# Weobe/plonky2-ecdsa

Hardware: AMD Instinct MI355X
Metric: secp256k1 ECDSA witness fills/sec at batch=2^16, 1/2/4/8 MI355X; bit-exact (higher is better)
Workload: dtype u64

## Files before the change

__graft_entry__.py:

```python
import os
import subprocess
import sys

ROOT = os.path.dirname(os.path.abspath(__file__))
sys.path.insert(0, ROOT)


def build() -> None:
    import plonky2_ecdsa_amd as p2e
    p2e.build(verbose=True)
    subprocess.check_call(["make", "-s", "-C", os.path.join(ROOT, "oracle"), "libp2e_oracle.so"])
    subprocess.check_call(["make", "-s", "-C", os.path.join(ROOT, "tests", "emu")])
    subprocess.check_call(["make", "-s", "-C", os.path.join(ROOT, "tests", "probe")])
    subprocess.check_call(["make", "-s", "-C", os.path.join(ROOT, "tests", "probe_hash")])
    p2e.lib()
    assert p2e.schedule_num_cols(p2e.PROGRAM_VERIFY) == p2e.VERIFY_COLS


def smoke() -> None:
    import numpy as np
    import torch
    import plonky2_ecdsa_amd as p2e
    sys.path.insert(0, os.path.join(ROOT, "oracle"))
    import oracle_c

    n = 64
    sigs = p2e.synth_signatures(seed=1, n=n)
    ctx = p2e.Context(device=0, phase_timing=True)
    dev = [torch.from_numpy(a).cuda() for a in sigs]
    cols, err, valid, bad = ctx.ecdsa_verify_witness_batch(*dev)
    torch.cuda.synchronize()
    assert bad == 0 and bool(valid.cpu().numpy().all()), "synthetic signatures must verify"
    ref_cols, ref_aux, ref_err, ref_flags = oracle_c.verify_witness_aux(*sigs)
    got = cols.cpu().numpy().view(np.uint64)
    assert np.array_equal(got, ref_cols), "GPU witness differs from the oracle"
    phases = ctx.last_phase_ms()
    aux, aerr, abad = ctx.aux_witness_batch(p2e.PROGRAM_VERIFY, dev[4], cols, n=n, ld=cols.stride(0))
    torch.cuda.synchronize()
    assert abad == 0 and np.array_equal(aux.cpu().numpy().view(np.uint64), ref_aux), "aux columns differ from the oracle"
    print(f"smoke ok: {n} fills x ({p2e.VERIFY_COLS} + {p2e.VERIFY_AUX_COLS}) columns bit-exact vs oracle; phases {phases}")


if __name__ == "__main__":
    build()
    if "--smoke" in sys.argv:
        smoke()
```

plonky2-ecdsa_amd/csrc/p2e_hip.hip:

```cpp
#include <hip/hip_runtime.h>

#include <algorithm>
#include <cstdio>
#include <cstdlib>
#include <cstring>
#include <memory>
#include <mutex>
#include <string>
#include <type_traits>
#include <vector>

#include "../../include/p2e.h"
#include "aux.hpp"
#include "consts.hpp"
#include "device_array.hpp"
#include "knobs.hpp"
#include "launch_plan.hpp"
#include "pipeline.hpp"
#include "prims.hpp"
#include "quad.hpp"
#include "schedule.hpp"
#include "curve_program.hpp"
#include "sign.hpp"
#include "recover.hpp"
#include "pmsm.hpp"
#include "hash.hpp"
#include "wire.hpp"

using namespace p2e;
using host::COMPACT_WIDE;

#ifndef P2E_PART
#define P2E_PART (-1)
#endif
#define P2E_HAS(p) (P2E_PART < 0 || P2E_PART == (p))

constexpr int BS = 256;

template <bool WIDE>
__device__ __forceinline__ size_t lane_sig(size_t first) {
    unsigned t = threadIdx.x;
    size_t base = first + (size_t)blockIdx.x * BS;
    if (WIDE) return base + (t & ~63u) + 2u * (t & 31u) + ((t >> 5) & 1u);
    return base + t;
}
template <int MODE> struct EmitOf;
template <> struct EmitOf<0> { typedef Emit type; };
template <> struct EmitOf<1> { typedef PairEmit type; };
template <> struct EmitOf<2> { typedef CompactEmit type; };
template <> struct EmitOf<3> { typedef CompactPairEmit type; };
template <> struct EmitOf<4> { typedef NullEmit type; };
#if P2E_HAS(1)
template <int MODE>
__global__ __launch_bounds__(BS) void k_scalar(Program G, Buffers B, size_t first) {
    size_t i = lane_sig<(MODE & 1) != 0>(first);
    if ((MODE & 1) || i < B.n) body_scalar<typename EmitOf<MODE>::type>(G, B, i);
}
__global__ __launch_bounds__(BS) void k_chains(Program G, Buffers B, int lo, int hi, int table_affine, int continue_prefix) {
    __builtin_amdgcn_s_setprio(3);
    size_t i = (size_t)blockIdx.x * BS + threadIdx.x;
#ifdef P2E_LDS_FBTAB
    constexpr int MAXW = 36;
    __shared__ Aff s_fb[MAXW * 16];
    const OpDesc first = load_op(B.ops, lo);
    const bool fb = first.kind != OP_DBL && ref_kind(first.ref2) == R_FBTAB && hi - lo <= MAXW;
    const u32 w0 = ref_id(first.ref2);
    if (fb) {
        const int nwin = (hi - lo) < (int)(FB_WINDOWS - w0) ? (hi - lo) : (int)(FB_WINDOWS - w0);
        const u32* src = reinterpret_cast<const u32*>(B.fbtab + (size_t)w0 * 16);
        u32* dst = reinterpret_cast<u32*>(s_fb);
        for (int k = threadIdx.x; k < nwin * 16 * 16; k += BS) dst[k] = src[k];
    }
    __syncthreads();
    if (i < B.n) body_chain_range(G, B, i, lo, hi, table_affine != 0, continue_prefix != 0, fb ? s_fb : nullptr, w0);
#else
    if (i < B.n) body_chain_range(G, B, i, lo, hi, table_affine != 0, continue_prefix != 0);
#endif
}
__global__ __launch_bounds__(BS) void k_chains_quad(Program G, Buffers B, int lo, int hi, int table_affine, int continue_prefix) {
    __builtin_amdgcn_s_setprio(3);
    const size_t g = (size_t)blockIdx.x * BS + threadIdx.x;
    const size_t i = g >> 2;
    if (i < B.n) body_chain_range_quad(G, B, i, (int)(g & 3), lo, hi, table_affine != 0, continue_prefix != 0);
}
__global__ __launch_bounds__(BS) void k_batch_inv_split(Program G, Buffers B, int lo, int hi, int have_prefix, int split_log2) {
    const size_t g = (size_t)blockIdx.x * BS + threadIdx.x;
    const size_t i = g >> split_log2;
    if (i < B.n) body_batch_inv_split(G, B, i, lo, hi, have_prefix != 0, (int)(g & ((1u << split_log2) - 1)), 1 << split_log2);
}
__global__ __launch_bounds__(BS) void k_chain_rows(Program G, Buffers B, int lo, int count) {
    __builtin_amdgcn_s_setprio(3);
    size_t i = (size_t)blockIdx.x * BS + threadIdx.x;
    if (i < B.n) body_chain_rows(G, B, i, lo, (int)gridDim.y, (int)blockIdx.y, count);
}
__global__ __launch_bounds__(BS) void k_batch_inv(Program G, Buffers B, int lo, int hi, int have_prefix) {
    size_t i = (size_t)blockIdx.x * BS + threadIdx.x;
    if (i < B.n) body_batch_inv(G, B, i, lo, hi, have_prefix != 0);
}
template <int MODE>
__global__ __launch_bounds__(BS) void k_expand(Program G, Buffers B, int lo, size_t first) {
#ifdef P2E_EXPAND_PRIO
    __builtin_amdgcn_s_setprio(P2E_EXPAND_PRIO);
#endif
    size_t i = lane_sig<(MODE & 1) != 0>(first);
#ifdef P2E_LDS_FBTAB
    __shared__ Aff s_fb[16];
    const OpDesc op0 = load_op(B.ops, lo + (int)blockIdx.y);
    const bool fb = op0.kind != OP_DBL && ref_kind(op0.ref2) == R_FBTAB;
    if (fb) reinterpret_cast<u32*>(s_fb)[threadIdx.x] = reinterpret_cast<const u32*>(B.fbtab + (size_t)ref_id(op0.ref2) * 16)[threadIdx.x];
    __syncthreads();
    if ((MODE & 1) || i < B.n) body_expand<typename EmitOf<MODE>::type>(G, B, i, lo + (int)blockIdx.y, fb ? s_fb : nullptr);
#else
    if ((MODE & 1) || i < B.n) body_expand<typename EmitOf<MODE>::type>(G, B, i, lo + (int)blockIdx.y);
#endif
}
template <int MODE>
__global__ __launch_bounds__(BS) void k_expand_runs(Program G, Buffers B, int it_first, int run_iters, int it_end, size_t first) {
#ifdef P2E_EXPAND_PRIO
    __builtin_amdgcn_s_setprio(P2E_EXPAND_PRIO);
#endif
    size_t i = lane_sig<(MODE & 1) != 0>(first);
    int it0 = it_first + (int)blockIdx.y * run_iters;
    int it1 = it0 + run_iters < it_end ? it0 + run_iters : it_end;
    if ((MODE & 1) || i < B.n) body_expand_run<typename EmitOf<MODE>::type>(G, B, i, it0, it1);
}
template <int MODE>
__global__ __launch_bounds__(BS) void k_expand_fb_run(Program G, Buffers B, int t_after, size_t first) {
    size_t i = lane_sig<(MODE & 1) != 0>(first);
    if ((MODE & 1) || i < B.n) body_expand_fb_run<typename EmitOf<MODE>::type>(G, B, i, t_after);
}
__global__ __launch_bounds__(BS) void k_verify_check(Program G, Buffers B) {
    size_t i = (size_t)blockIdx.x * BS + threadIdx.x;
    if (i < B.n) body_verify_check(G, B, i);
}
#endif
template <int MODE> struct AuxEmitOf;
template <> struct AuxEmitOf<0> { typedef Emit type; };
template <> struct AuxEmitOf<1> { typedef PairEmit type; };
template <> struct AuxEmitOf<2> { typedef Emit32 type; };
template <> struct AuxEmitOf<3> { typedef PairEmit32 type; };
#if P2E_HAS(0)
template <int MODE>
__global__ __launch_bounds__(BS) void k_aux(AuxArgs A, size_t first) {
    size_t i = lane_sig<(MODE & 1) != 0>(first);
    if ((MODE & 1) || i < A.n) body_aux<typename AuxEmitOf<MODE>::type>(A, (int)blockIdx.y, i);
}
template <int MODE>
__global__ __launch_bounds__(BS) void k_gate(GateArgs A, size_t first) {
    size_t i = lane_sig<(MODE & 1) != 0>(first);
    if ((MODE & 1) || i < A.n) body_gate<typename AuxEmitOf<MODE>::type>(A, (int)blockIdx.y, i);
}
template <int MODE>
__global__ __launch_bounds__(BS) void k_ux(UxArgs A, size_t first) {
    size_t i = lane_sig<(MODE & 1) != 0>(first);
    if ((MODE & 1) || i < A.n) body_ux<typename AuxEmitOf<MODE>::type>(A, (int)blockIdx.y, i);
}
template <int MODE>
__global__ __launch_bounds__(BS) void k_gate_compact(GateArgs A, size_t first) {
    size_t i = lane_sig<(MODE & 1) != 0>(first);
    if ((MODE & 1) || i < A.n) body_gate<typename AuxEmitOf<MODE>::type, true>(A, (int)blockIdx.y, i);
}
template <int MODE>
__global__ __launch_bounds__(BS) void k_ux_compact(UxArgs A, size_t first) {
    size_t i = lane_sig<(MODE & 1) != 0>(first);
    if ((MODE & 1) || i < A.n) body_ux<typename AuxEmitOf<MODE>::type, true>(A, (int)blockIdx.y, i);
}
#endif
static __global__ __launch_bounds__(BS) void k_finalize(const u32* err32, const uint8_t* valid8, uint8_t* err_out,
                                                 uint8_t* valid_out, size_t n, unsigned long long* counter) {
    size_t i = (size_t)blockIdx.x * BS + threadIdx.x;
    bool bad = false;
    if (i < n) {
        u32 e = err32[i];
        bad = e != 0;
        if (err_out) err_out[i] = (uint8_t)e;
        if (valid_out) valid_out[i] = bad ? 0 : valid8[i];
    }
    unsigned long long m = __ballot(bad);
// ... 2510 lines not shown
```

plonky2-ecdsa_amd/csrc/pipeline.hpp:

```cpp
#pragma once
#include "ec29.hpp"
#include "wit.hpp"

namespace p2e {

enum OpKind : uint8_t { OP_ADD = 0, OP_DBL = 1, OP_CADD = 2 };
enum RefKind : uint32_t { R_SLOT = 0, R_CONST = 1, R_DYN = 2, R_FBTAB = 3, R_MSMTAB = 4, R_SELSLOT = 5 };
enum OpFlags : uint8_t { F_Z1ONE = 1, F_Z2ONE = 2, F_CHECK_R = 4, F_NO_AFFINE = 8 };
P2E_HD constexpr u32 make_ref(u32 kind, u32 id) { return (kind << 24) | id; }
P2E_HD constexpr u32 ref_kind(u32 r) { return r >> 24; }
P2E_HD constexpr u32 ref_id(u32 r) { return r & 0xFFFFFFu; }
constexpr uint16_t DYN_CONST_BIT = 0x8000;
constexpr uint16_t SRC_FB_BIT = 0x4000, SRC_SEL_BIT = 0x2000, SRC_ID_MASK = 0x1FFF;

struct OpDesc {
    uint8_t kind;
    uint8_t flags;
    uint16_t cadd_idx;
    u32 ref1, ref2;
    u32 col;
};
static_assert(sizeof(OpDesc) == 16, "load_op reads a descriptor as one 16-byte word");
P2E_HD OpDesc load_op(const OpDesc* ops, int t) {
#if defined(__HIP_DEVICE_COMPILE__)
// ... 219 lines not shown
    return B.fbtab[window * 16 + digit];
}

struct ChainState {
    Jac out, p1;
    uint16_t out_id, p1_id;
    U256 acc;
};
P2E_HD Jac jac_select3(bool c1, const Jac& a, bool c2, const Jac& b, const Jac& c) {
    Jac r;
    r.X = u256_select(c1, a.X, u256_select(c2, b.X, c.X));
    r.Y = u256_select(c1, a.Y, u256_select(c2, b.Y, c.Y));
    r.Z = u256_select(c1, a.Z, u256_select(c2, b.Z, c.Z));
    return r;
}
template <class CV = Secp256k1, bool GENERIC = false>
P2E_HD void body_chain_op(const Program& G, const Buffers& B, size_t i, int t, bool table_affine, ChainState& st,
                          const Aff* lds_fb = nullptr, u32 lds_w0 = 0) {
    typedef typename CV::Fp F;
    const OpDesc op = load_op(B.ops, t);
    size_t o = (size_t)t * B.n + i;
    JacW res;
    uint16_t src1 = resolve_src(G, B, i, op.ref1);
    const bool from_out = src1 == st.out_id, from_p1 = src1 == st.p1_id;
    Jac p1 = st.out;
    if (!(from_out || from_p1)) p1 = load_jac_src(B, i, src1, (op.flags & F_Z1ONE) != 0);
    p1 = jac_select3(from_out, st.out, from_p1, st.p1, p1);
    B.src[(size_t)(2 * t) * B.n + i] = src1;
    if (op.kind == OP_DBL) {
        res = jac_dbl_cv<CV>(p1);
    } else {
        Jac p2;
        u32 digit = 1;
        uint16_t src2;
        bool z2one = (op.flags & F_Z2ONE) != 0;
        if (GENERIC && ref_kind(op.ref2) == R_SELSLOT) {
            digit = B.dig2[(size_t)(ref_id(op.ref2) >> 12) * B.n + i];
            src2 = (uint16_t)(ref_id(op.ref2) & 0xFFFu);
            p2 = load_jac_src(B, i, src2, z2one);
        } else if (ref_kind(op.ref2) == R_FBTAB) {
            Aff a = load_fbtab(B, i, ref_id(op.ref2), digit, lds_fb, lds_w0);
            p2 = jac_from_aff(a);
            src2 = (uint16_t)(SRC_FB_BIT | (ref_id(op.ref2) * 16 + digit));
        } else {
            const bool tab = ref_kind(op.ref2) == R_MSMTAB;
            if (tab) digit = B.dig2[(size_t)ref_id(op.ref2) * B.n + i];
            src2 = resolve_src(G, B, i, op.ref2);
            if (tab && table_affine) {
                p2 = jac_from_aff(load_aff_src(B, i, src2));
                z2one = true;
            } else {
                p2 = load_jac_src(B, i, src2, (op.flags & F_Z2ONE) != 0);
            }
        }
        B.src[(size_t)(2 * t + 1) * B.n + i] = (uint16_t)(src2 | (digit != 0 ? SRC_SEL_BIT : 0));
        if ((op.flags & F_Z1ONE) && z2one)
            res = jac_add_cv<CV, true, true>(p1, p2);
        else if (z2one)
            res = jac_add_cv<CV, false, true>(p1, p2);
        else if (op.flags & F_Z1ONE)
            res = jac_add_cv<CV, true, false>(p1, p2);
        else
            res = jac_add_cv<CV, false, false>(p1, p2);
        if (op.kind == OP_CADD) B.dyn[(size_t)op.cadd_idx * B.n + i] = digit != 0 ? (uint16_t)t : src1;
    }
    if (!(op.flags & F_NO_AFFINE)) {
        B.PX[o] = res.p.X;
        B.PY[o] = res.p.Y;
    }
    B.PZ[o] = res.p.Z;
    B.PW[o] = res.W;
    B.PREF[o] = st.acc;
    U256 z = res.p.Z;
    if (u256_is_zero(z)) {
        err_or(&B.err[i], ERR_INVERSE_OF_ZERO);
        z = u256_small(1);
    }
    st.acc = fe_mul<F>(st.acc, z);
    st.p1 = p1;
    st.p1_id = (op.flags & F_Z1ONE) ? (uint16_t)0xFFFF : src1;
    st.out = res.p;
    st.out_id = (uint16_t)t;
}
struct ChainState29 {
    JacL out, p1;
    uint16_t out_id, p1_id;
    F29 acc;
};
template <bool GENERIC = false>
P2E_HD void body_chain_op29(const Program& G, const Buffers& B, size_t i, int t, bool table_affine, ChainState29& st,
                            const Aff* lds_fb = nullptr, u32 lds_w0 = 0) {
    const OpDesc op = load_op(B.ops, t);
    size_t o = (size_t)t * B.n + i;
    JacWL res;
    uint16_t src1 = resolve_src(G, B, i, op.ref1);
    const bool from_out = src1 == st.out_id, from_p1 = src1 == st.p1_id;
    JacL p1 = st.out;
    if (!(from_out || from_p1)) p1 = jacl_from(load_jac_src(B, i, src1, (op.flags & F_Z1ONE) != 0));
    p1 = jacl_select3(from_out, st.out, from_p1, st.p1, p1);
    B.src[(size_t)(2 * t) * B.n + i] = src1;
    if (op.kind == OP_DBL) {
        res = jac_dbl29(p1);
    } else {
        Jac p2w;
        u32 digit = 1;
        uint16_t src2;
        bool z2one = (op.flags & F_Z2ONE) != 0;
        if (GENERIC && ref_kind(op.ref2) == R_SELSLOT) {
            digit = B.dig2[(size_t)(ref_id(op.ref2) >> 12) * B.n + i];
            src2 = (uint16_t)(ref_id(op.ref2) & 0xFFFu);
            p2w = load_jac_src(B, i, src2, z2one);
        } else if (ref_kind(op.ref2) == R_FBTAB) {
            Aff a = load_fbtab(B, i, ref_id(op.ref2), digit, lds_fb, lds_w0);
            p2w = jac_from_aff(a);
            src2 = (uint16_t)(SRC_FB_BIT | (ref_id(op.ref2) * 16 + digit));
        } else {
            const bool tab = ref_kind(op.ref2) == R_MSMTAB;
            if (tab) digit = B.dig2[(size_t)ref_id(op.ref2) * B.n + i];
            src2 = resolve_src(G, B, i, op.ref2);
            if (tab && table_affine) {
                p2w = jac_from_aff(load_aff_src(B, i, src2));
                z2one = true;
            } else {
                p2w = load_jac_src(B, i, src2, (op.flags & F_Z2ONE) != 0);
            }
        }
        B.src[(size_t)(2 * t + 1) * B.n + i] = (uint16_t)(src2 | (digit != 0 ? SRC_SEL_BIT : 0));
        const JacL p2 = jacl_from(p2w);
        if ((op.flags & F_Z1ONE) && z2one)
            res = jac_add29<true, true>(p1, p2);
        else if (z2one)
            res = jac_add29<false, true>(p1, p2);
        else if (op.flags & F_Z1ONE)
            res = jac_add29<true, false>(p1, p2);
        else
            res = jac_add29<false, false>(p1, p2);
        if (op.kind == OP_CADD) B.dyn[(size_t)op.cadd_idx * B.n + i] = digit != 0 ? (uint16_t)t : src1;
    }
    if (!(op.flags & F_NO_AFFINE)) {
        B.PX[o] = f29_canon_call(res.p.X);
        B.PY[o] = f29_canon_call(res.p.Y);
    }
    const U256 zc = f29_canon_call(res.p.Z);
    B.PZ[o] = zc;
    B.PW[o] = f29_canon_call(res.W);
    B.PREF[o] = f29_canon_call(st.acc);
    const bool z_zero = u256_is_zero(zc);
    if (z_zero) err_or(&B.err[i], ERR_INVERSE_OF_ZERO);
    st.acc = f29_mul_call(st.acc, f29_select(z_zero, f29_small(1), res.p.Z));
    st.p1 = p1;
    st.p1_id = (op.flags & F_Z1ONE) ? (uint16_t)0xFFFF : src1;
    st.out = res.p;
    st.out_id = (uint16_t)t;
}
P2E_HD ChainState29 chain_state29_init(const U256& acc) {
    ChainState29 st;
    st.out_id = st.p1_id = 0xFFFF;
    st.out.X = st.out.Y = st.out.Z = st.p1.X = st.p1.Y = st.p1.Z = f29_small(0);
    st.acc = f29_from_u256(acc);
    return st;
}
template <class CV = Secp256k1>
P2E_HD U256 range_product(const Buffers& B, size_t i, int last) {
    size_t o = (size_t)last * B.n + i;
    U256 z = B.PZ[o];
    if (u256_is_zero(z)) z = u256_small(1);
    return fe_mul<typename CV::Fp>(B.PREF[o], z);
}
template <class CV = Secp256k1, bool GENERIC = false>
P2E_HD void body_chain_range(const Program& G, const Buffers& B, size_t i, int lo, int hi, bool table_affine,
                             bool continue_prefix, const Aff* lds_fb = nullptr, u32 lds_w0 = 0) {
    if (LazyLimbs<CV>::available) {
        ChainState29 st = chain_state29_init(continue_prefix ? range_product<CV>(B, i, lo - 1) : u256_small(1));
        for (int t = lo; t < hi; t++) body_chain_op29<GENERIC>(G, B, i, t, table_affine, st, lds_fb, lds_w0);
        return;
    }
    ChainState st;
    st.out_id = st.p1_id = 0xFFFF;
    st.out.X = st.out.Y = st.out.Z = st.p1.X = st.p1.Y = st.p1.Z = u256_zero();
    st.acc = continue_prefix ? range_product<CV>(B, i, lo - 1) : u256_small(1);
    for (int t = lo; t < hi; t++) body_chain_op<CV, GENERIC>(G, B, i, t, table_affine, st, lds_fb, lds_w0);
}

P2E_HD void body_chain_rows(const Program& G, const Buffers& B, size_t i, int lo, int rows, int row, int count) {
    ChainState29 st = chain_state29_init(u256_small(1));
    for (int j = 0; j < count; j++) body_chain_op29(G, B, i, lo + row + j * rows, false, st);
}

template <class CV = Secp256k1>
P2E_HD void body_verify_check(const Program& G, const Buffers& B, size_t i, int last_op) {
    typedef typename CV::Fp F;
    const size_t o = (size_t)last_op * B.n + i;
    const U256 r = load_packed(B.r, i), X = B.PX[o], Z = B.PZ[o];
    const bool r_lt_p = !geq_mod<F>(r.w);
    if (!(r_lt_p && !u256_is_zero(Z) && u256_eq(fe_mul<F>(r, fe_sqr<F>(Z)), X))) B.valid[i] = 0;
}
P2E_HD void body_verify_check(const Program& G, const Buffers& B, size_t i) {
    body_verify_check<Secp256k1>(G, B, i, G.chain_end[2] - 1);
}

P2E_HD void body_batch_inv29(const Buffers& B, size_t i, int t0, int t1, bool have_prefix, bool uniform_t) {
    U256 accw;
    if (have_prefix) {
        accw = range_product<Secp256k1>(B, i, t1 - 1);
    } else {
        F29 acc = f29_small(1);
        for (int t = t0; t < t1; t++) {
            const size_t o = (size_t)t * B.n + i;
            U256 z = B.PZ[o];
            if (u256_is_zero(z)) z = u256_small(1);
            B.PREF[o] = f29_canon_call(acc);
            acc = f29_mul_call(acc, f29_from_u256(z));
        }
        accw = f29_canon_call(acc);
    }
    F29 inv = f29_from_u256(fe_inv<ModP>(accw));
    struct In {
        U256 z, pref, w, x, y;
        uint8_t flags;
    };
    auto flags_of = [&](int t) { return uniform_t ? load_op(B.ops, t < t0 ? t0 : t).flags : B.ops[t < t0 ? t0 : t].flags; };
    auto fetch = [&](int t, uint8_t fl) {
        In r;
        const size_t o = (size_t)(t < t0 ? t0 : t) * B.n + i;
        const bool aff = !(fl & F_NO_AFFINE);
        r.z = B.PZ[o];
        r.pref = B.PREF[o];
        r.w = B.PW[o];
        r.x = *(aff ? &B.PX[o] : &B.PZ[o]);
        r.y = *(aff ? &B.PY[o] : &B.PZ[o]);
        r.flags = fl;
        return r;
    };
    uint8_t f_nxt = flags_of(t1 - 2);
    In cur = fetch(t1 - 1, flags_of(t1 - 1));
    for (int t = t1 - 1; t >= t0; t--) {
        const uint8_t f_n2 = flags_of(t - 2);
        const In nxt = fetch(t - 1, f_nxt);
        const size_t o = (size_t)t * B.n + i;
        const U256 z = u256_select(u256_is_zero(cur.z), u256_small(1), cur.z);
        const F29 zi = f29_mul_call(inv, f29_from_u256(cur.pref));
        inv = f29_mul_call(inv, f29_from_u256(z));
        B.PW[o] = f29_canon_call(f29_mul_call(f29_from_u256(cur.w), zi));
        if (!(cur.flags & F_NO_AFFINE)) {
            const F29 zi2 = f29_sqr_call(zi);
            const F29 zi3 = f29_mul_call(zi2, zi);
            B.AX[o] = f29_canon_call(f29_mul_call(f29_from_u256(cur.x), zi2));
            B.AY[o] = f29_canon_call(f29_mul_call(f29_from_u256(cur.y), zi3));
        }
        cur = nxt;
        f_nxt = f_n2;
    }
}
template <class CV = Secp256k1>
P2E_HD void body_batch_inv(const Program& G, const Buffers& B, size_t i, int t0, int t1, bool have_prefix, bool uniform_t = true) {
    (void)G;
    typedef typename CV::Fp F;
    if (LazyLimbs<CV>::available) {
        body_batch_inv29(B, i, t0, t1, have_prefix, uniform_t);
        return;
    }
    U256 acc;
    if (have_prefix) {
        acc = range_product<CV>(B, i, t1 - 1);
    } else {
        acc = u256_small(1);
        for (int t = t0; t < t1; t++) {
            size_t o = (size_t)t * B.n + i;
            U256 z = B.PZ[o];
            if (u256_is_zero(z)) z = u256_small(1);
            B.PREF[o] = acc;
            acc = fe_mul<F>(acc, z);
        }
    }
    U256 inv = fe_inv<F>(acc);
    for (int t = t1 - 1; t >= t0; t--) {
        size_t o = (size_t)t * B.n + i;
        U256 z = B.PZ[o];
        if (u256_is_zero(z)) z = u256_small(1);
        U256 zi = fe_mul<F>(inv, B.PREF[o]);
        inv = fe_mul<F>(inv, z);
        B.PW[o] = fe_mul<F>(B.PW[o], zi);
        const uint8_t flags = uniform_t ? load_op(B.ops, t).flags : B.ops[t].flags;
        if (!(flags & F_NO_AFFINE)) {
            U256 zi2 = fe_sqr<F>(zi);
            U256 zi3 = fe_mul<F>(zi2, zi);
            B.AX[o] = fe_mul<F>(B.PX[o], zi2);
            B.AY[o] = fe_mul<F>(B.PY[o], zi3);
        }
    }
}

template <class E, class CV = Secp256k1>
P2E_HD Aff wit_curve_add(E& e, const Aff& p1, const Aff& p2, const U256& vinv, uint8_t& err) {
    U256 u = wit_sub<typename CV::Fp>(e, p2.y, p1.y);
    U256 v = wit_sub<typename CV::Fp>(e, p2.x, p1.x);
    wit_inv_given<typename CV::Fp>(e, v, vinv, err);
    U256 s = wit_mul<typename CV::Fp>(e, u, vinv, err);
    U256 s2 = wit_mul<typename CV::Fp>(e, s, s, err);
    U256 xs = wit_add<typename CV::Fp>(e, p2.x, p1.x);
    Aff r;
    r.x = wit_sub<typename CV::Fp>(e, s2, xs);
    U256 xd = wit_sub<typename CV::Fp>(e, p1.x, r.x);
    U256 pr = wit_mul<typename CV::Fp>(e, s, xd, err);
    r.y = wit_sub<typename CV::Fp>(e, pr, p1.y);
    return r;
}
template <class E, class CV = Secp256k1>
P2E_HD Aff wit_curve_double(E& e, const Aff& p, const U256& vinv, uint8_t& err) {
    U256 dy = wit_add<typename CV::Fp>(e, p.y, p.y);
    wit_inv_given<typename CV::Fp>(e, dy, vinv, err);
    U256 xx = wit_mul<typename CV::Fp>(e, p.x, p.x, err);
    U256 summ[4] = {xx, xx, xx, CV::a()};
    U256 t = wit_add_many<typename CV::Fp, 4>(e, summ);
    U256 l = wit_mul<typename CV::Fp>(e, t, vinv, err);
    U256 l2 = wit_mul<typename CV::Fp>(e, l, l, err);
    U256 xd2 = wit_add<typename CV::Fp>(e, p.x, p.x);
    Aff r;
    r.x = wit_sub<typename CV::Fp>(e, l2, xd2);
    U256 xdf = wit_sub<typename CV::Fp>(e, p.x, r.x);
    U256 lx = wit_mul<typename CV::Fp>(e, l, xdf, err);
    r.y = wit_sub<typename CV::Fp>(e, lx, p.y);
    return r;
}
template <class E, class CV = Secp256k1>
P2E_HD void body_expand(const Program& G, const Buffers& B, size_t i, int t, const Aff* lds_fb = nullptr) {
    const OpDesc op = load_op(B.ops, t);
    uint8_t err = 0;
    E e = E::at(B.sink, i, op.col);
    const uint16_t s1 = B.src[(size_t)(2 * t) * B.n + i];
    const uint16_t s2 = op.kind == OP_DBL ? (uint16_t)0 : B.src[(size_t)(2 * t + 1) * B.n + i];
    U256 vinv = B.PW[(size_t)t * B.n + i];
    Aff p1 = load_aff_src(B, i, s1);
    if (op.kind == OP_DBL) {
// ... 78 lines not shown
```

plonky2-ecdsa_amd/csrc/quad.hpp:

```cpp
#pragma once
#include "pipeline.hpp"
#include "quad29.hpp"

namespace p2e {

#if defined(__HIP_DEVICE_COMPILE__)
template <int J>
__device__ __forceinline__ U256 quad_bcast(const U256& v) {
    U256 r;
    P2E_UNROLL
    for (int k = 0; k < 8; k++)
        r.w[k] = (u32)__builtin_amdgcn_mov_dpp((int)v.w[k], J * 0x55 , 0xF, 0xF, true);
    return r;
}
#endif

template <int USED, bool SQR, class CV = Secp256k1>
P2E_HD void quad_level(int role, const U256& a0, const U256& b0, const U256& a1, const U256& b1, const U256& a2,
                       const U256& b2, const U256& a3, const U256& b3, U256& r0, U256& r1, U256& r2, U256& r3) {
#if defined(__HIP_DEVICE_COMPILE__)
    U256 A = a0, B = b0;
    if (USED > 1) {
        A = u256_select(role == 1, a1, A);
        if (!SQR) B = u256_select(role == 1, b1, B);
// ... 103 lines not shown
P2E_HD QuadRes jac_dbl_quad_cv(int role, const Jac& p, const U256& acc) {
    typedef typename CV::Fp F;
    if (CV::kAZero) return jac_dbl_quad(role, p, acc);
    U256 a, b, yz, zz, c, t0, w, d0, f, y0;
    quad_level<4, false, CV>(role, p.X, p.X, p.Y, p.Y, p.Y, p.Z, p.Z, p.Z, a, b, yz, zz);
    const U256 z3 = fe_add<F>(yz, yz);
    quad_level<3, true, CV>(role, b, b, fe_add<F>(p.X, b), b, zz, b, zz, b, c, t0, w, d0);
    const U256 t = fe_sub<F>(fe_sub<F>(t0, a), c);
    const U256 d = fe_add<F>(t, t);
    const U256 e1 = fe_sub<F>(a, w);
    const U256 e = fe_add<F>(fe_add<F>(e1, e1), e1);
    QuadRes o;
    o.z3_zero = u256_is_zero(z3);
    const U256 zfix = u256_select(o.z3_zero, u256_small(1), z3);
    quad_level<3, false, CV>(role, e, e, acc, zfix, z3, z3, z3, z3, f, o.acc, o.zz3, d0);
    o.res.p.X = fe_sub<F>(f, fe_add<F>(d, d));
    const U256 c2 = fe_add<F>(c, c), c4 = fe_add<F>(c2, c2), c8 = fe_add<F>(c4, c4);
    quad_level<1, false, CV>(role, e, fe_sub<F>(d, o.res.p.X), e, e, e, e, e, e, y0, d0, d0, d0);
    o.res.p.Y = fe_sub<F>(y0, c8);
    o.res.p.Z = z3;
    o.res.W = w;
    o.zz1 = zz;
    return o;
}
template <class CV, bool Z1ONE, bool Z2ONE>
P2E_HD QuadRes jac_add_quad_cv(int role, const Jac& p1, bool have_zz1, const U256& zz1_in, const Jac& p2, const U256& acc) {
    typedef typename CV::Fp F;
    if (CV::kAZero) return jac_add_quad<Z1ONE, Z2ONE>(role, p1, have_zz1, zz1_in, p2, acc);
    U256 zz1 = zz1_in, zz2, z12, z1c, z2c, u1 = p1.X, u2 = p2.X, s1 = p1.Y, s2 = p2.Y, d0, d1;
    if (!Z1ONE && !Z2ONE) {
        quad_level<3, false, CV>(role, p1.Z, p1.Z, p2.Z, p2.Z, p1.Z, p2.Z, p1.Z, p1.Z, zz1, zz2, z12, d0);
    } else if (!Z1ONE) {
        if (!have_zz1) quad_level<1, true, CV>(role, p1.Z, p1.Z, p1.Z, p1.Z, p1.Z, p1.Z, p1.Z, p1.Z, zz1, d0, d1, d0);
    } else if (!Z2ONE) {
        quad_level<1, true, CV>(role, p2.Z, p2.Z, p2.Z, p2.Z, p2.Z, p2.Z, p2.Z, p2.Z, zz2, d0, d1, d0);
    }
    if (!Z1ONE && !Z2ONE) {
        quad_level<4, false, CV>(role, zz1, p1.Z, zz2, p2.Z, p1.X, zz2, p2.X, zz1, z1c, z2c, u1, u2);
    } else if (!Z1ONE) {
        quad_level<2, false, CV>(role, zz1, p1.Z, p2.X, zz1, zz1, zz1, zz1, zz1, z1c, u2, d0, d1);
    } else if (!Z2ONE) {
        quad_level<2, false, CV>(role, zz2, p2.Z, p1.X, zz2, zz2, zz2, zz2, zz2, z2c, u1, d0, d1);
    }
    const U256 h = fe_sub<F>(u2, u1);
    U256 h2, z3;
    if (!Z1ONE && !Z2ONE) {
        quad_level<4, false, CV>(role, p1.Y, z2c, p2.Y, z1c, h, h, z12, h, s1, s2, h2, z3);
    } else if (!Z1ONE) {
        quad_level<3, false, CV>(role, p2.Y, z1c, h, h, p1.Z, h, h, h, s2, h2, z3, d0);
    } else if (!Z2ONE) {
        quad_level<3, false, CV>(role, p1.Y, z2c, h, h, p2.Z, h, h, h, s1, h2, z3, d0);
    } else {
        quad_level<1, true, CV>(role, h, h, h, h, h, h, h, h, h2, d0, d1, d0);
        z3 = h;
    }
    const U256 r = fe_sub<F>(s2, s1);
    U256 h3, v, r2;
    QuadRes o;
    if (!Z1ONE && !Z2ONE) {
        quad_level<4, false, CV>(role, h2, h, u1, h2, r, r, z1c, z2c, h3, v, r2, o.res.W);
    } else {
        quad_level<3, false, CV>(role, h2, h, u1, h2, r, r, r, r, h3, v, r2, d0);
        o.res.W = Z1ONE ? (Z2ONE ? u256_small(1) : z2c) : z1c;
    }
    o.res.p.X = fe_sub<F>(fe_sub<F>(r2, h3), fe_add<F>(v, v));
    o.z3_zero = u256_is_zero(z3);
    const U256 zfix = u256_select(o.z3_zero, u256_small(1), z3);
    U256 t1, t2;
    quad_level<4, false, CV>(role, r, fe_sub<F>(v, o.res.p.X), s1, h3, acc, zfix, z3, z3, t1, t2, o.acc, o.zz3);
    o.res.p.Y = fe_sub<F>(t1, t2);
    o.res.p.Z = z3;
    o.zz1 = zz1;
    return o;
}

struct ChainStateQ {
    Jac out, p1;
    U256 out_zz, p1_zz;
    uint16_t out_id, p1_id;
    uint16_t dyn_idx, dyn_val;
    U256 acc;
};

P2E_HD void settle(U256& v) {
#if defined(__HIP_DEVICE_COMPILE__)
    asm volatile("" : "+v"(v.w[0]), "+v"(v.w[1]), "+v"(v.w[2]), "+v"(v.w[3]), "+v"(v.w[4]), "+v"(v.w[5]), "+v"(v.w[6]), "+v"(v.w[7]));
#else
    (void)v;
#endif
}
P2E_HD void settle(u32& v) {
#if defined(__HIP_DEVICE_COMPILE__)
    asm volatile("" : "+v"(v));
#else
    (void)v;
#endif
}

P2E_HD void quad_store_op(const Buffers& B, size_t i, int role, int t, uint8_t flags, const QuadRes& q, const U256& acc_before) {
    const size_t o = (size_t)t * B.n + i;
    const int r = (flags & F_NO_AFFINE) ? (role | 2) : role;
    uintptr_t bx = (uintptr_t)B.PX, by = (uintptr_t)B.PY, bz = (uintptr_t)B.PZ, bw = (uintptr_t)B.PW;
#if defined(__HIP_DEVICE_COMPILE__)
    asm volatile("" : "+s"(bx), "+s"(by), "+s"(bz), "+s"(bw));
#endif
    U256* const dst = (U256*)(r == 0 ? bx : r == 1 ? by : r == 2 ? bz : bw);
    const U256 val = u256_select(r == 0, q.res.p.X, u256_select(r == 1, q.res.p.Y, u256_select(r == 2, q.res.p.Z, q.res.W)));
    dst[o] = val;
    B.PREF[o] = acc_before;
    if (q.z3_zero) err_or(&B.err[i], ERR_INVERSE_OF_ZERO);
}

P2E_HD void quad_store_op29(const Buffers& B, size_t i, int role, int t, uint8_t flags, const QuadRes29& q) {
    const size_t o = (size_t)t * B.n + i;
    const bool no_affine = (flags & F_NO_AFFINE) != 0;
    uintptr_t bx = (uintptr_t)B.PX, bp = (uintptr_t)B.PREF, bz = (uintptr_t)B.PZ, bw = (uintptr_t)B.PW;
#if defined(__HIP_DEVICE_COMPILE__)
    asm volatile("" : "+s"(bx), "+s"(bp), "+s"(bz), "+s"(bw));
#endif
    U256* const dst = (U256*)(role == 1 ? bp : role == 3 ? bw : (role == 0 && !no_affine) ? bx : bz);
    dst[o] = q.mine;
    if (!no_affine) B.PY[o] = f29_canon(q.p.Y);
    if (q.z3_zero) err_or(&B.err[i], ERR_INVERSE_OF_ZERO);
}

struct P1Sel {
    uint16_t src1;
    Jac p1;
    bool have_zz1;
    U256 zz1;
};
P2E_HD P1Sel quad_first_operand(const Program& G, const Buffers& B, size_t i, const OpDesc& op, const ChainStateQ& st) {
    P1Sel r;
    u32 src1;
    if (ref_kind(op.ref1) == R_DYN && ref_id(op.ref1) == st.dyn_idx) {
        src1 = st.dyn_val;
    } else {
        src1 = resolve_src(G, B, i, op.ref1);
        settle(src1);
    }
    r.src1 = (uint16_t)src1;
    const bool from_out = r.src1 == st.out_id, from_p1 = r.src1 == st.p1_id;
    Jac p1 = st.out;
    if (!(from_out || from_p1)) {
        p1 = load_jac_src(B, i, r.src1, (op.flags & F_Z1ONE) != 0);
        settle(p1.X);
        settle(p1.Y);
        settle(p1.Z);
    }
    r.p1 = jac_select3(from_out, st.out, from_p1, st.p1, p1);
    r.have_zz1 = from_out || from_p1;
    r.zz1 = u256_select(from_out, st.out_zz, st.p1_zz);
    return r;
}

P2E_HD void body_chain_op_quad(const Program& G, const Buffers& B, size_t i, int role, int t, const OpDesc& op, bool table_affine,
                               const P1Sel& s1, ChainStateQ& st) {
    const uint16_t src1 = s1.src1;
    const Jac& p1 = s1.p1;
    if (role == 0) B.src[(size_t)(2 * t) * B.n + i] = src1;
    QuadRes q;
    if (op.kind == OP_DBL) {
        q = jac_dbl_quad(role, p1, st.acc);
    } else {
        Jac p2;
        u32 digit = 1;
        uint16_t src2;
        bool z2one = (op.flags & F_Z2ONE) != 0;
        {
            if (ref_kind(op.ref2) == R_FBTAB) {
                Aff a = load_fbtab(B, i, ref_id(op.ref2), digit);
                p2 = jac_from_aff(a);
                src2 = (uint16_t)(SRC_FB_BIT | (ref_id(op.ref2) * 16 + digit));
            } else {
                const bool tab = ref_kind(op.ref2) == R_MSMTAB;
                if (tab) digit = B.dig2[(size_t)ref_id(op.ref2) * B.n + i];
                src2 = resolve_src(G, B, i, op.ref2);
                if (tab && table_affine) {
                    p2 = jac_from_aff(load_aff_src(B, i, src2));
                    z2one = true;
// ... 298 lines not shown
```

Measured before the change: 6.054 million.

## Add specialized per-lane chain paths for MSM iterations and fixed-base windows

Adds lane-specialized chain kernels for MSM loop iterations (double, double, conditional add) and fixed-base window runs. Both prefetch the next digit and source one iteration ahead and keep the running point in registers instead of resolving and reloading operands per op. Store code is moved into a shared helper, stores are reordered after the arithmetic, and the batch-inverse back pass drops its one-ahead prefetch. Also raises the wave priority of k_batch_inv. This adds code size and register pressure, and the change in load scheduling may not pay off.

```diff
diff --git a/__graft_entry__.py b/__graft_entry__.py
--- a/__graft_entry__.py
+++ b/__graft_entry__.py
@@ -11,6 +11,7 @@
     p2e.build(verbose=True)
     subprocess.check_call(["make", "-s", "-C", os.path.join(ROOT, "oracle"), "libp2e_oracle.so"])
     subprocess.check_call(["make", "-s", "-C", os.path.join(ROOT, "tests", "emu")])
+    subprocess.check_call(["make", "-s", "-C", os.path.join(ROOT, "tests", "emu_lane")])
     subprocess.check_call(["make", "-s", "-C", os.path.join(ROOT, "tests", "probe")])
     subprocess.check_call(["make", "-s", "-C", os.path.join(ROOT, "tests", "probe_hash")])
     p2e.lib()
diff --git a/plonky2-ecdsa_amd/csrc/p2e_hip.hip b/plonky2-ecdsa_amd/csrc/p2e_hip.hip
--- a/plonky2-ecdsa_amd/csrc/p2e_hip.hip
+++ b/plonky2-ecdsa_amd/csrc/p2e_hip.hip
@@ -94,6 +94,7 @@
     if (i < B.n) body_chain_rows(G, B, i, lo, (int)gridDim.y, (int)blockIdx.y, count);
 }
 __global__ __launch_bounds__(BS) void k_batch_inv(Program G, Buffers B, int lo, int hi, int have_prefix) {
+    __builtin_amdgcn_s_setprio(1);
     size_t i = (size_t)blockIdx.x * BS + threadIdx.x;
     if (i < B.n) body_batch_inv(G, B, i, lo, hi, have_prefix != 0);
 }
diff --git a/plonky2-ecdsa_amd/csrc/pipeline.hpp b/plonky2-ecdsa_amd/csrc/pipeline.hpp
--- a/plonky2-ecdsa_amd/csrc/pipeline.hpp
+++ b/plonky2-ecdsa_amd/csrc/pipeline.hpp
@@ -330,18 +330,35 @@
     uint16_t out_id, p1_id;
     F29 acc;
 };
+P2E_HD void chain_store_op29(const Buffers& B, size_t i, int t, uint8_t flags, const JacWL& res, F29& acc) {
+    const size_t o = (size_t)t * B.n + i;
+    const U256 pref = f29_canon_call(acc);
+    const U256 zc = f29_canon_call(res.p.Z);
+    const bool z_zero = u256_is_zero(zc);
+    acc = f29_mul_call(acc, f29_select(z_zero, f29_small(1), res.p.Z));
+    const U256 wc = f29_canon_call(res.W);
+    if (!(flags & F_NO_AFFINE)) {
+        const U256 xc = f29_canon_call(res.p.X);
+        const U256 yc = f29_canon_call(res.p.Y);
+        B.PX[o] = xc;
+        B.PY[o] = yc;
+    }
+    B.PZ[o] = zc;
+    B.PW[o] = wc;
+    B.PREF[o] = pref;
+    if (z_zero) err_or(&B.err[i], ERR_INVERSE_OF_ZERO);
+}
 template <bool GENERIC = false>
 P2E_HD void body_chain_op29(const Program& G, const Buffers& B, size_t i, int t, bool table_affine, ChainState29& st,
                             const Aff* lds_fb = nullptr, u32 lds_w0 = 0) {
     const OpDesc op = load_op(B.ops, t);
-    size_t o = (size_t)t * B.n + i;
     JacWL res;
     uint16_t src1 = resolve_src(G, B, i, op.ref1);
     const bool from_out = src1 == st.out_id, from_p1 = src1 == st.p1_id;
     JacL p1 = st.out;
     if (!(from_out || from_p1)) p1 = jacl_from(load_jac_src(B, i, src1, (op.flags & F_Z1ONE) != 0));
     p1 = jacl_select3(from_out, st.out, from_p1, st.p1, p1);
-    B.src[(size_t)(2 * t) * B.n + i] = src1;
+    uint16_t src2_sel = 0, dyn_val = 0;
     if (op.kind == OP_DBL) {
         res = jac_dbl29(p1);
     } else {
@@ -368,7 +385,7 @@
                 p2w = load_jac_src(B, i, src2, (op.flags & F_Z2ONE) != 0);
             }
         }
-        B.src[(size_t)(2 * t + 1) * B.n + i] = (uint16_t)(src2 | (digit != 0 ? SRC_SEL_BIT : 0));
+        src2_sel = (uint16_t)(src2 | (digit != 0 ? SRC_SEL_BIT : 0));
         const JacL p2 = jacl_from(p2w);
         if ((op.flags & F_Z1ONE) && z2one)
             res = jac_add29<true, true>(p1, p2);
@@ -378,19 +395,12 @@
             res = jac_add29<true, false>(p1, p2);
         else
             res = jac_add29<false, false>(p1, p2);
-        if (op.kind == OP_CADD) B.dyn[(size_t)op.cadd_idx * B.n + i] = digit != 0 ? (uint16_t)t : src1;
-    }
-    if (!(op.flags & F_NO_AFFINE)) {
-        B.PX[o] = f29_canon_call(res.p.X);
-        B.PY[o] = f29_canon_call(res.p.Y);
-    }
-    const U256 zc = f29_canon_call(res.p.Z);
-    B.PZ[o] = zc;
-    B.PW[o] = f29_canon_call(res.W);
-    B.PREF[o] = f29_canon_call(st.acc);
-    const bool z_zero = u256_is_zero(zc);
-    if (z_zero) err_or(&B.err[i], ERR_INVERSE_OF_ZERO);
-    st.acc = f29_mul_call(st.acc, f29_select(z_zero, f29_small(1), res.p.Z));
+        dyn_val = digit != 0 ? (uint16_t)t : src1;
+    }
+    chain_store_op29(B, i, t, op.flags, res, st.acc);
+    B.src[(size_t)(2 * t) * B.n + i] = src1;
+    if (op.kind != OP_DBL) B.src[(size_t)(2 * t + 1) * B.n + i] = src2_sel;
+    if (op.kind == OP_CADD) B.dyn[(size_t)op.cadd_idx * B.n + i] = dyn_val;
     st.p1 = p1;
     st.p1_id = (op.flags & F_Z1ONE) ? (uint16_t)0xFFFF : src1;
     st.out = res.p;
@@ -410,11 +420,147 @@
     if (u256_is_zero(z)) z = u256_small(1);
     return fe_mul<typename CV::Fp>(B.PREF[o], z);
 }
+P2E_HD void settle(U256& v) {
+#if defined(__HIP_DEVICE_COMPILE__)
+    asm volatile("" : "+v"(v.w[0]), "+v"(v.w[1]), "+v"(v.w[2]), "+v"(v.w[3]), "+v"(v.w[4]), "+v"(v.w[5]), "+v"(v.w[6]), "+v"(v.w[7]));
+#else
+    (void)v;
+#endif
+}
+P2E_HD void settle(u32& v) {
+#if defined(__HIP_DEVICE_COMPILE__)
+    asm volatile("" : "+v"(v));
+#else
+    (void)v;
+#endif
+}
+
+P2E_HD JacL lane_first_operand(const Program& G, const Buffers& B, size_t i, const OpDesc& op, uint16_t& src1) {
+    u32 s = resolve_src(G, B, i, op.ref1);
+    settle(s);
+    src1 = (uint16_t)s;
+    Jac w = load_jac_src(B, i, src1, (op.flags & F_Z1ONE) != 0);
+    settle(w.X);
+    settle(w.Y);
+    settle(w.Z);
+    return jacl_from(w);
+}
+P2E_HD void body_msm_iters_lane(const Program& G, const Buffers& B, size_t i, int it0, int it1, JacL& c, uint16_t& cur_id, F29& acc) {
+    const int lb = G.msm_loop_begin;
+    auto digit_row = [&](int it) { return (size_t)ref_id(load_op(B.ops, lb + 3 * (it < it1 ? it : it1 - 1) + 2).ref2); };
+    struct Sel {
+        u32 digit;
+        u32 src;
+    };
+    auto sel_of = [&](int it) {
+        Sel s;
+        const size_t row = digit_row(it);
+        s.digit = B.dig2[row * B.n + i];
+        s.src = B.msrc[row * B.n + i];
+        return s;
+    };
+    Sel s_cur = sel_of(it0);
+    settle(s_cur.digit);
+    settle(s_cur.src);
+    for (int it = it0; it < it1; it++) {
+        const int t = lb + 3 * it;
+        const bool is_const = (s_cur.src & DYN_CONST_BIT) != 0;
+        const size_t po = (size_t)(s_cur.src & SRC_ID_MASK) * B.n + i;
+        const Aff* cp = &B.cpts[is_const ? (s_cur.src & SRC_ID_MASK) : 0];
+        const U256 p2x = *(is_const ? &cp->x : &B.AX[po]);
+        const U256 p2y = *(is_const ? &cp->y : &B.AY[po]);
+        const Sel s_nxt = sel_of(it + 1);
+        const OpDesc o0 = load_op(B.ops, t), o1 = load_op(B.ops, t + 1), o2 = load_op(B.ops, t + 2);
+        for (int k = 0; k < 2; k++) {
+            const JacWL d = jac_dbl29(c);
+            chain_store_op29(B, i, t + k, k ? o1.flags : o0.flags, d, acc);
+            B.src[(size_t)(2 * (t + k)) * B.n + i] = cur_id;
+            c = d.p;
+            cur_id = (uint16_t)(t + k);
+        }
+        JacL p2;
+        p2.X = f29_from_u256(p2x);
+        p2.Y = f29_from_u256(p2y);
+        p2.Z = f29_small(1);
+        const JacWL a = jac_add29<false, true>(c, p2);
+        const bool take = s_cur.digit != 0;
+        const uint16_t dyn_val = take ? (uint16_t)(t + 2) : cur_id;
+        chain_store_op29(B, i, t + 2, o2.flags, a, acc);
+        B.src[(size_t)(2 * (t + 2)) * B.n + i] = cur_id;
+        B.src[(size_t)(2 * (t + 2) + 1) * B.n + i] = (uint16_t)(s_cur.src | (take ? SRC_SEL_BIT : 0));
+        B.dyn[(size_t)o2.cadd_idx * B.n + i] = dyn_val;
+        c.X = f29_select(take, a.p.X, c.X);
+        c.Y = f29_select(take, a.p.Y, c.Y);
+        c.Z = f29_select(take, a.p.Z, c.Z);
+        cur_id = dyn_val;
+        s_cur = s_nxt;
+    }
+}
+P2E_HD void body_fb_windows_lane(const Buffers& B, size_t i, int t0, int count, JacL& c, uint16_t& cur_id, F29& acc) {
+    const int t1 = t0 + count;
+    auto window_of = [&](int t) { return ref_id(load_op(B.ops, t < t1 ? t : t1 - 1).ref2); };
+    auto digit_of_op = [&](int t) { return (u32)B.dig4[(size_t)window_of(t) * B.n + i]; };
+    u32 d_cur = digit_of_op(t0);
+    settle(d_cur);
+    for (int t = t0; t < t1; t++) {
+        const OpDesc o = load_op(B.ops, t);
+        const Aff p2a = B.fbtab[ref_id(o.ref2) * 16 + d_cur];
+        const u32 d_nxt = digit_of_op(t + 1);
+        JacL p2;
+        p2.X = f29_from_u256(p2a.x);
+        p2.Y = f29_from_u256(p2a.y);
+        p2.Z = f29_small(1);
+        const JacWL a = jac_add29<false, true>(c, p2);
+        const bool take = d_cur != 0;
+        const uint16_t dyn_val = take ? (uint16_t)t : cur_id;
+        chain_store_op29(B, i, t, o.flags, a, acc);
+        B.src[(size_t)(2 * t) * B.n + i] = cur_id;
+        B.src[(size_t)(2 * t + 1) * B.n + i] = (uint16_t)(SRC_FB_BIT | (ref_id(o.ref2) * 16 + d_cur) | (take ? SRC_SEL_BIT : 0));
+        B.dyn[(size_t)o.cadd_idx * B.n + i] = dyn_val;
+        c.X = f29_select(take, a.p.X, c.X);
+        c.Y = f29_select(take, a.p.Y, c.Y);
+        c.Z = f29_select(take, a.p.Z, c.Z);
+        cur_id = dyn_val;
+        d_cur = d_nxt;
+    }
+}
+P2E_HD void body_chain_range_lane(const Program& G, const Buffers& B, size_t i, int lo, int hi, bool table_affine, ChainState29& st) {
+    const int lb = G.msm_loop_begin, le = lb + 3 * G.msm_loop_iters;
+    int t = lo;
+    const OpDesc op = load_op(B.ops, lo);
+    const bool msm_iter = table_affine && lo >= lb && lo + 3 <= le && lo + 3 <= hi && (lo - lb) % 3 == 0;
+    const bool fb_window = op.kind == OP_CADD && ref_kind(op.ref2) == R_FBTAB;
+    if (msm_iter || fb_window) {
+        uint16_t cur_id;
+        JacL cur = lane_first_operand(G, B, i, op, cur_id);
+        if (msm_iter) {
+            const int it0 = (lo - lb) / 3, hi_it = ((hi < le ? hi : le) - lb) / 3;
+            body_msm_iters_lane(G, B, i, it0, hi_it, cur, cur_id, st.acc);
+            t += 3 * (hi_it - it0);
+        } else {
+            int count = 1;
+            while (t + count < hi) {
+                const OpDesc nx = load_op(B.ops, t + count);
+                if (!(nx.kind == OP_CADD && ref_kind(nx.ref2) == R_FBTAB)) break;
+                count++;
+            }
+            body_fb_windows_lane(B, i, t, count, cur, cur_id, st.acc);
+            t += count;
+        }
+        st.out = cur;
+        st.out_id = cur_id;
+    }
+    for (; t < hi; t++) body_chain_op29(G, B, i, t, table_affine, st);
+}
 template <class CV = Secp256k1, bool GENERIC = false>
 P2E_HD void body_chain_range(const Program& G, const Buffers& B, size_t i, int lo, int hi, bool table_affine,
                              bool continue_prefix, const Aff* lds_fb = nullptr, u32 lds_w0 = 0) {
     if (LazyLimbs<CV>::available) {
         ChainState29 st = chain_state29_init(continue_prefix ? range_product<CV>(B, i, lo - 1) : u256_small(1));
+        if (!GENERIC && !lds_fb) {
+            body_chain_range_lane(G, B, i, lo, hi, table_affine, st);
+            return;
+        }
         for (int t = lo; t < hi; t++) body_chain_op29<GENERIC>(G, B, i, t, table_affine, st, lds_fb, lds_w0);
         return;
     }
@@ -452,8 +598,9 @@
             const size_t o = (size_t)t * B.n + i;
             U256 z = B.PZ[o];
             if (u256_is_zero(z)) z = u256_small(1);
-            B.PREF[o] = f29_canon_call(acc);
+            const U256 pref = f29_canon_call(acc);
             acc = f29_mul_call(acc, f29_from_u256(z));
+            B.PREF[o] = pref;
         }
         accw = f29_canon_call(acc);
     }
@@ -475,24 +622,25 @@
         r.flags = fl;
         return r;
     };
-    uint8_t f_nxt = flags_of(t1 - 2);
-    In cur = fetch(t1 - 1, flags_of(t1 - 1));
+    uint8_t f_cur = flags_of(t1 - 1);
     for (int t = t1 - 1; t >= t0; t--) {
-        const uint8_t f_n2 = flags_of(t - 2);
-        const In nxt = fetch(t - 1, f_nxt);
+        const uint8_t f_nxt = flags_of(t - 1);
+        const In cur = fetch(t, f_cur);
         const size_t o = (size_t)t * B.n + i;
         const U256 z = u256_select(u256_is_zero(cur.z), u256_small(1), cur.z);
         const F29 zi = f29_mul_call(inv, f29_from_u256(cur.pref));
         inv = f29_mul_call(inv, f29_from_u256(z));
-        B.PW[o] = f29_canon_call(f29_mul_call(f29_from_u256(cur.w), zi));
+        const U256 vinv = f29_canon_call(f29_mul_call(f29_from_u256(cur.w), zi));
         if (!(cur.flags & F_NO_AFFINE)) {
             const F29 zi2 = f29_sqr_call(zi);
             const F29 zi3 = f29_mul_call(zi2, zi);
-            B.AX[o] = f29_canon_call(f29_mul_call(f29_from_u256(cur.x), zi2));
-            B.AY[o] = f29_canon_call(f29_mul_call(f29_from_u256(cur.y), zi3));
-        }
-        cur = nxt;
-        f_nxt = f_n2;
+            const U256 ax = f29_canon_call(f29_mul_call(f29_from_u256(cur.x), zi2));
+            const U256 ay = f29_canon_call(f29_mul_call(f29_from_u256(cur.y), zi3));
+            B.AX[o] = ax;
+            B.AY[o] = ay;
+        }
+        B.PW[o] = vinv;
+        f_cur = f_nxt;
     }
 }
 template <class CV = Secp256k1>
diff --git a/plonky2-ecdsa_amd/csrc/quad.hpp b/plonky2-ecdsa_amd/csrc/quad.hpp
--- a/plonky2-ecdsa_amd/csrc/quad.hpp
+++ b/plonky2-ecdsa_amd/csrc/quad.hpp
@@ -209,20 +209,6 @@
     U256 acc;
 };
 
-P2E_HD void settle(U256& v) {
-#if defined(__HIP_DEVICE_COMPILE__)
-    asm volatile("" : "+v"(v.w[0]), "+v"(v.w[1]), "+v"(v.w[2]), "+v"(v.w[3]), "+v"(v.w[4]), "+v"(v.w[5]), "+v"(v.w[6]), "+v"(v.w[7]));
-#else
-    (void)v;
-#endif
-}
-P2E_HD void settle(u32& v) {
-#if defined(__HIP_DEVICE_COMPILE__)
-    asm volatile("" : "+v"(v));
-#else
-    (void)v;
-#endif
-}
 
 P2E_HD void quad_store_op(const Buffers& B, size_t i, int role, int t, uint8_t flags, const QuadRes& q, const U256& acc_before) {
     const size_t o = (size_t)t * B.n + i;
```

Result: no change. 6.059 million, median of 2 (+0.1%).

## Prefetch fixed-base table points and carry dyn ids across chain ops

Applied to the files above, without the earlier changes.

Adds a register ring that loads the fixed-base digit and table point for upcoming windows one op ahead, so the loads overlap the current point addition. It also carries the last conditional-add result id in registers to skip re-reading the dyn buffer, and moves the per-op stores after the arithmetic. The batch-inversion loop gets a configurable prefetch depth (default 1) and likewise defers its stores. This raises register pressure and may lower occupancy.

```diff
diff --git a/plonky2-ecdsa_amd/csrc/pipeline.hpp b/plonky2-ecdsa_amd/csrc/pipeline.hpp
--- a/plonky2-ecdsa_amd/csrc/pipeline.hpp
+++ b/plonky2-ecdsa_amd/csrc/pipeline.hpp
@@ -325,23 +325,67 @@
     st.out = res.p;
     st.out_id = (uint16_t)t;
 }
+#ifndef P2E_FB_AHEAD
+#define P2E_FB_AHEAD 1
+#endif
+constexpr int FB_AHEAD = P2E_FB_AHEAD;
+static_assert(FB_AHEAD >= 1, "the ring holds at least the next window");
 struct ChainState29 {
     JacL out, p1;
     uint16_t out_id, p1_id;
     F29 acc;
+    int32_t dyn_idx;
+    uint16_t dyn_id;
+    bool fb_on;
+    int32_t fb_next, fb_first, fb_last;
+    u32 fb_dig[FB_AHEAD + 1];
+    Aff fb_pt[FB_AHEAD];
 };
+P2E_HD u32 fb_ring_window(const ChainState29& st, int k) {
+    const int w = st.fb_next + k;
+    return (u32)(w < st.fb_first ? st.fb_first : w > st.fb_last ? st.fb_last : w);
+}
+P2E_HD Aff fbtab_point(const Buffers& B, u32 window, u32 digit, const Aff* lds_fb, u32 lds_w0) {
+    if (lds_fb) return lds_fb[(window - lds_w0) * 16 + digit];
+    return B.fbtab[window * 16 + digit];
+}
+P2E_HD void fb_ring_start(const Program& G, const Buffers& B, size_t i, int lo, int hi, ChainState29& st, const Aff* lds_fb,
+                          u32 lds_w0) {
+    if (G.fb_begin < 0) return;
+    const int nwin = G.fb_windows < FB_WINDOWS ? G.fb_windows : FB_WINDOWS;
+    const int first = lo > G.fb_begin ? lo - G.fb_begin : 0, last = (hi - G.fb_begin < nwin ? hi - G.fb_begin : nwin) - 1;
+    if (first > last) return;
+    st.fb_on = true;
+    st.fb_next = lo - G.fb_begin;
+    st.fb_first = first;
+    st.fb_last = last;
+    P2E_UNROLL
+    for (int k = 0; k <= FB_AHEAD; k++) st.fb_dig[k] = B.dig4[(size_t)fb_ring_window(st, k) * B.n + i];
+    P2E_UNROLL
+    for (int k = 0; k < FB_AHEAD; k++) st.fb_pt[k] = fbtab_point(B, fb_ring_window(st, k), st.fb_dig[k], lds_fb, lds_w0);
+}
+P2E_HD void fb_ring_advance(const Buffers& B, size_t i, ChainState29& st, const Aff* lds_fb, u32 lds_w0) {
+    st.fb_next++;
+    P2E_UNROLL
+    for (int k = 0; k < FB_AHEAD; k++) st.fb_dig[k] = st.fb_dig[k + 1];
+    P2E_UNROLL
+    for (int k = 0; k + 1 < FB_AHEAD; k++) st.fb_pt[k] = st.fb_pt[k + 1];
+    st.fb_dig[FB_AHEAD] = B.dig4[(size_t)fb_ring_window(st, FB_AHEAD) * B.n + i];
+    st.fb_pt[FB_AHEAD - 1] = fbtab_point(B, fb_ring_window(st, FB_AHEAD - 1), st.fb_dig[FB_AHEAD - 1], lds_fb, lds_w0);
+}
 template <bool GENERIC = false>
 P2E_HD void body_chain_op29(const Program& G, const Buffers& B, size_t i, int t, bool table_affine, ChainState29& st,
                             const Aff* lds_fb = nullptr, u32 lds_w0 = 0) {
     const OpDesc op = load_op(B.ops, t);
     size_t o = (size_t)t * B.n + i;
     JacWL res;
-    uint16_t src1 = resolve_src(G, B, i, op.ref1);
+    const bool carried = ref_kind(op.ref1) == R_DYN && (int32_t)ref_id(op.ref1) == st.dyn_idx;
+    uint16_t src1 = carried ? st.dyn_id : resolve_src(G, B, i, op.ref1);
     const bool from_out = src1 == st.out_id, from_p1 = src1 == st.p1_id;
     JacL p1 = st.out;
     if (!(from_out || from_p1)) p1 = jacl_from(load_jac_src(B, i, src1, (op.flags & F_Z1ONE) != 0));
     p1 = jacl_select3(from_out, st.out, from_p1, st.p1, p1);
-    B.src[(size_t)(2 * t) * B.n + i] = src1;
+    uint16_t src2_sel = 0, dyn_id = 0;
     if (op.kind == OP_DBL) {
         res = jac_dbl29(p1);
     } else {
@@ -354,7 +398,14 @@
             src2 = (uint16_t)(ref_id(op.ref2) & 0xFFFu);
             p2w = load_jac_src(B, i, src2, z2one);
         } else if (ref_kind(op.ref2) == R_FBTAB) {
-            Aff a = load_fbtab(B, i, ref_id(op.ref2), digit, lds_fb, lds_w0);
+            const int w = (int)ref_id(op.ref2);
+            Aff a;
+            if (st.fb_on && w == st.fb_next && w >= st.fb_first && w <= st.fb_last) {
+                a = st.fb_pt[0];
+                digit = st.fb_dig[0];
+            } else {
+                a = load_fbtab(B, i, (u32)w, digit, lds_fb, lds_w0);
+            }
             p2w = jac_from_aff(a);
             src2 = (uint16_t)(SRC_FB_BIT | (ref_id(op.ref2) * 16 + digit));
         } else {
@@ -368,7 +419,7 @@
                 p2w = load_jac_src(B, i, src2, (op.flags & F_Z2ONE) != 0);
             }
         }
-        B.src[(size_t)(2 * t + 1) * B.n + i] = (uint16_t)(src2 | (digit != 0 ? SRC_SEL_BIT : 0));
+        src2_sel = (uint16_t)(src2 | (digit != 0 ? SRC_SEL_BIT : 0));
         const JacL p2 = jacl_from(p2w);
         if ((op.flags & F_Z1ONE) && z2one)
             res = jac_add29<true, true>(p1, p2);
@@ -378,26 +429,48 @@
             res = jac_add29<true, false>(p1, p2);
         else
             res = jac_add29<false, false>(p1, p2);
-        if (op.kind == OP_CADD) B.dyn[(size_t)op.cadd_idx * B.n + i] = digit != 0 ? (uint16_t)t : src1;
-    }
-    if (!(op.flags & F_NO_AFFINE)) {
-        B.PX[o] = f29_canon_call(res.p.X);
-        B.PY[o] = f29_canon_call(res.p.Y);
+        dyn_id = digit != 0 ? (uint16_t)t : src1;
+    }
+    const bool affine = !(op.flags & F_NO_AFFINE);
+    U256 xc = u256_zero(), yc = u256_zero();
+    if (affine) {
+        xc = f29_canon_call(res.p.X);
+        yc = f29_canon_call(res.p.Y);
     }
     const U256 zc = f29_canon_call(res.p.Z);
-    B.PZ[o] = zc;
-    B.PW[o] = f29_canon_call(res.W);
-    B.PREF[o] = f29_canon_call(st.acc);
+    const U256 wc = f29_canon_call(res.W);
+    const U256 prefc = f29_canon_call(st.acc);
     const bool z_zero = u256_is_zero(zc);
-    if (z_zero) err_or(&B.err[i], ERR_INVERSE_OF_ZERO);
     st.acc = f29_mul_call(st.acc, f29_select(z_zero, f29_small(1), res.p.Z));
     st.p1 = p1;
     st.p1_id = (op.flags & F_Z1ONE) ? (uint16_t)0xFFFF : src1;
     st.out = res.p;
     st.out_id = (uint16_t)t;
+    if (st.fb_on) fb_ring_advance(B, i, st, lds_fb, lds_w0);
+    B.src[(size_t)(2 * t) * B.n + i] = src1;
+    if (op.kind != OP_DBL) B.src[(size_t)(2 * t + 1) * B.n + i] = src2_sel;
+    if (op.kind == OP_CADD) {
+        B.dyn[(size_t)op.cadd_idx * B.n + i] = dyn_id;
+        st.dyn_idx = (int32_t)op.cadd_idx;
+        st.dyn_id = dyn_id;
+    }
+    if (affine) {
+        B.PX[o] = xc;
+        B.PY[o] = yc;
+    }
+    B.PZ[o] = zc;
+    B.PW[o] = wc;
+    B.PREF[o] = prefc;
+    if (z_zero) err_or(&B.err[i], ERR_INVERSE_OF_ZERO);
 }
 P2E_HD ChainState29 chain_state29_init(const U256& acc) {
     ChainState29 st;
+    st.dyn_idx = -1;
+    st.dyn_id = 0;
+    st.fb_on = false;
+    st.fb_next = st.fb_first = st.fb_last = 0;
+    for (int k = 0; k <= FB_AHEAD; k++) st.fb_dig[k] = 0;
+    for (int k = 0; k < FB_AHEAD; k++) st.fb_pt[k].x = st.fb_pt[k].y = u256_zero();
     st.out_id = st.p1_id = 0xFFFF;
     st.out.X = st.out.Y = st.out.Z = st.p1.X = st.p1.Y = st.p1.Z = f29_small(0);
     st.acc = f29_from_u256(acc);
@@ -415,6 +488,7 @@
                              bool continue_prefix, const Aff* lds_fb = nullptr, u32 lds_w0 = 0) {
     if (LazyLimbs<CV>::available) {
         ChainState29 st = chain_state29_init(continue_prefix ? range_product<CV>(B, i, lo - 1) : u256_small(1));
+        fb_ring_start(G, B, i, lo, hi, st, lds_fb, lds_w0);
         for (int t = lo; t < hi; t++) body_chain_op29<GENERIC>(G, B, i, t, table_affine, st, lds_fb, lds_w0);
         return;
     }
@@ -442,6 +516,11 @@
     body_verify_check<Secp256k1>(G, B, i, G.chain_end[2] - 1);
 }
 
+#ifndef P2E_BINV_DEPTH
+#define P2E_BINV_DEPTH 1
+#endif
+constexpr int BINV_DEPTH = P2E_BINV_DEPTH;
+static_assert(BINV_DEPTH >= 1 && BINV_DEPTH <= 4, "request depth of body_batch_inv29");
 P2E_HD void body_batch_inv29(const Buffers& B, size_t i, int t0, int t1, bool have_prefix, bool uniform_t) {
     U256 accw;
     if (have_prefix) {
@@ -475,24 +554,37 @@
         r.flags = fl;
         return r;
     };
-    uint8_t f_nxt = flags_of(t1 - 2);
+    constexpr int D = BINV_DEPTH;
     In cur = fetch(t1 - 1, flags_of(t1 - 1));
+    In pend[D];
+    P2E_UNROLL
+    for (int k = 0; k + 1 < D; k++) pend[k] = fetch(t1 - 2 - k, flags_of(t1 - 2 - k));
+    uint8_t f_req = flags_of(t1 - 1 - D);
     for (int t = t1 - 1; t >= t0; t--) {
-        const uint8_t f_n2 = flags_of(t - 2);
-        const In nxt = fetch(t - 1, f_nxt);
+        const uint8_t f_n2 = flags_of(t - 1 - D);
         const size_t o = (size_t)t * B.n + i;
         const U256 z = u256_select(u256_is_zero(cur.z), u256_small(1), cur.z);
         const F29 zi = f29_mul_call(inv, f29_from_u256(cur.pref));
         inv = f29_mul_call(inv, f29_from_u256(z));
-        B.PW[o] = f29_canon_call(f29_mul_call(f29_from_u256(cur.w), zi));
-        if (!(cur.flags & F_NO_AFFINE)) {
+        const U256 vinv = f29_canon_call(f29_mul_call(f29_from_u256(cur.w), zi));
+        const bool affine = !(cur.flags & F_NO_AFFINE);
+        U256 ax = u256_zero(), ay = u256_zero();
+        if (affine) {
             const F29 zi2 = f29_sqr_call(zi);
             const F29 zi3 = f29_mul_call(zi2, zi);
-            B.AX[o] = f29_canon_call(f29_mul_call(f29_from_u256(cur.x), zi2));
-            B.AY[o] = f29_canon_call(f29_mul_call(f29_from_u256(cur.y), zi3));
-        }
-        cur = nxt;
-        f_nxt = f_n2;
+            ax = f29_canon_call(f29_mul_call(f29_from_u256(cur.x), zi2));
+            ay = f29_canon_call(f29_mul_call(f29_from_u256(cur.y), zi3));
+        }
+        pend[D - 1] = fetch(t - D, f_req);
+        B.PW[o] = vinv;
+        if (affine) {
+            B.AX[o] = ax;
+            B.AY[o] = ay;
+        }
+        cur = pend[0];
+        P2E_UNROLL
+        for (int k = 0; k + 1 < D; k++) pend[k] = pend[k + 1];
+        f_req = f_n2;
     }
 }
 template <class CV = Secp256k1>
```

Result: no change. 6.056 million before, 6.086 million after, median of 6 (+0.5%).
